# catid/siamese

Measured on AMD Instinct MI355X. Metric: device-resident GB/s encode+decode, 1400B pkts @20% loss; % HBM peak, higher is better.
Workload: dtype u8

## Files before the change

include/siamese_gpu.h:

```cpp
#ifndef SIAMESE_GPU_H
#define SIAMESE_GPU_H

#include "siamese.h"
#include <stddef.h>

#ifdef __cplusplus
extern "C" {
#endif

typedef struct SgpuEncoderImpl { int impl; }* SgpuEncoder;
typedef struct SgpuDecoderImpl { int impl; }* SgpuDecoder;

typedef struct SgpuRecoveryPacket
{
    const unsigned char* DeviceData;
    unsigned DataBytes;
    unsigned FooterBytes;
    unsigned char Footer[8];
    unsigned char Head[4];
    void* Producer;
} SgpuRecoveryPacket;

SIAMESE_EXPORT int sgpu_init(int device);

// ... 205 lines not shown
SIAMESE_EXPORT SiameseResult sgpu_decoders_ack_frames(const SgpuDecoder* decoders, unsigned count,
                                                      const unsigned* flows, unsigned byteLimit, void* deviceDst,
                                                      size_t stride, unsigned* deviceLens,
                                                      SiameseResult* results ,
                                                      unsigned* queuedOut);
SIAMESE_EXPORT SiameseResult sgpu_encoder_retransmit_frames(SgpuEncoder encoder, unsigned flow, unsigned maxPackets,
                                                            void* deviceDst, size_t stride, unsigned maxRows,
                                                            unsigned* deviceLens,
                                                            unsigned* packetNumsOut ,
                                                            unsigned* rowsOut, unsigned* framesOut);

#define SGPU_ROW_TRUNCATED       3
#define SGPU_PACKED_ACKS_DROPPED 0x20000000u

SIAMESE_EXPORT size_t sgpu_frames_duplex_bytes(unsigned count, unsigned maxFrames, unsigned ackSlots,
                                               unsigned ackBytes);
SIAMESE_EXPORT size_t sgpu_frames_duplex_slots(unsigned count, unsigned maxFrames);
SIAMESE_EXPORT long long sgpu_frames_scan_duplex(const void* deviceRows, size_t stride, const unsigned* deviceLens,
                                                 unsigned count, unsigned maxFrames, unsigned ackSlots,
                                                 unsigned ackBytes, void* pinnedOut);
SIAMESE_EXPORT SiameseResult sgpu_frames_recv_duplex(const SgpuDecoder* decoders, unsigned decoderCount,
                                                     const SgpuEncoder* encoders, unsigned encoderCount,
                                                     const void* heads, unsigned maxFrames, unsigned ackSlots,
                                                     unsigned ackBytes, const void* deviceRows, size_t stride,
                                                     unsigned count,
                                                     SiameseResult* results ,
                                                     unsigned* nextExpectedOut ,
                                                     unsigned* acceptedOut);

SIAMESE_EXPORT void sgpu_timing(int enable, int reset, double* execMs, double* totalMs);
SIAMESE_EXPORT void sgpu_timing_kernels(double* msOut, unsigned count);
SIAMESE_EXPORT void sgpu_engine_stats(uint64_t* out15);
SIAMESE_EXPORT void sgpu_engine_stats_ex(uint64_t* out, unsigned count);
SIAMESE_EXPORT void sgpu_measure_unique(int on);

SIAMESE_EXPORT uint64_t sgpu_arena_bytes(void);
SIAMESE_EXPORT int sgpu_arena_reserve(size_t bytes);

#ifdef __cplusplus
}
#endif

#endif
```

siamese_amd/csrc/backend.h:

```cpp
#pragma once

#include "ops.h"
#include <cstddef>
#include <cstdint>

namespace sgpu {

bool be_init(int device, const char** err);
const char* be_name();

void* be_dev_alloc(size_t bytes);
void be_dev_free(void* p);
void* be_host_alloc(size_t bytes);
void* be_host_alloc_mapped(size_t bytes);
void* be_host_device_ptr(void* host);
void be_host_free(void* p);

void be_h2d(void* dst, const void* src, size_t bytes);
void be_d2h(void* dst, const void* src, size_t bytes);
void be_memset(void* dst, int value, size_t bytes);
struct BeCopy
{
    uint64_t dst, src;
    uint64_t bytes;
// ... 5 lines not shown
struct BeIngest
{
    const IngestDesc* descs;
    uint32_t count;
    uint32_t maxBytes;
    const uint32_t* blocks = nullptr;
    uint32_t nblocks = 0;
};
void be_launch_ingest(const BeIngest& ingest);
void be_launch_exec(const void* stream, const ExecItem* items, uint32_t count, uint64_t* acct,
                    const uint32_t* results, uint32_t maxWindow);
uint32_t be_exec_stage_cap();
void be_launch_ldpc(const LdpcItem* items, uint32_t count, uint64_t* acct, const uint32_t* gates = nullptr,
                    const uint32_t* results = nullptr);
void be_launch_solve(const SolveDesc* solves, const SolveRow* rows, const uint8_t* coef, uint32_t* results,
                     const SolveItem* items, uint32_t count, uint32_t maxRows, uint64_t* acct,
                     uint32_t solveBegin, uint32_t solveCount);

struct BeGe
{
    const GeDesc* descs;
    const uint8_t* in;
    uint32_t count;
    uint32_t* results;
    const SolveRow* rowsIn;
    SolveRow* rows;
    uint8_t* coef;
    uint32_t maxRows, maxCols;
};
enum class GePlace
{
    kCodecStream,
    kSideStream,
};
void be_launch_ge(const BeGe& ge, GePlace place, const BeCopy& head = BeCopy{0, 0, 0});
void be_side_upload_ingest(const BeCopy& rest, const BeIngest& ingest);
void be_join_ge();

void be_launch_deliver(const DeliverItem* items, uint32_t count, uint32_t maxStride);
void be_launch_frame(const FrameItem* items, uint32_t count, uint32_t maxStride);
void be_launch_relay(const RelayItem* items, uint32_t count, uint32_t maxStride);
void be_launch_pack(const PackJob* jobs, uint32_t jobCount, const PackItem* items, uint32_t count, PlanRec* plan,
                    uint32_t maxStride);
void be_launch_concat(const ConcatJob* jobs, uint32_t jobCount, const ConcatItem* items, uint32_t count,
                      ConcatRec* recs, uint32_t maxBytes);

bool be_sync();

void* be_fence();
bool be_fence_wait(void* fence, unsigned spinUs, bool sleepPoll);

void* be_stage_h2d(void* dst, const void* src, size_t bytes);
void be_wait_mark(void* mark);
void be_mark_release(void* mark);
bool be_gather(const IngestDesc* descsHost, void* descsDev, uint32_t count, const void* devStage,
               void* hostOut, size_t bytes, void** packed, void** landed);
bool be_scan_rows(const void* rows, uint64_t stride, const uint32_t* lens, uint32_t count, void* devStage,
                  void* hostOut, void** packed, void** landed);
bool be_walk_rows(const void* rows, uint64_t stride, const uint32_t* lens, uint32_t count, uint32_t maxFrames,
                  void* devStage, void* hostOut, void** packed, void** landed);
bool be_ackwalk_rows(const void* rows, uint64_t stride, const uint32_t* lens, uint32_t count, uint32_t maxFrames,
                     uint32_t ackSlots, uint32_t ackBytes, void* devStage, void* hostOut, void** packed,
                     void** landed);
bool be_dense_rows(const void* rows, uint64_t stride, const uint32_t* lens, uint32_t count, uint32_t maxFrames,
                   uint32_t maxRecords, void* devStage, void* hostOut, void** packed, void** landed);
bool be_mark_sync(void* mark);
// ... 29 lines not shown
```

siamese_amd/csrc/backend_hip.hip:

```cpp
#include <hip/hip_runtime.h>

#include "backend.h"
#include "codedef.h"
#include "placement.h"
#include "pool.h"
#include "gf.h"

#include <algorithm>
#include <cctype>
#include <chrono>
#include <cstdlib>
#include <cstdio>
#include <string>
#include <type_traits>
#include <cstring>
#include <ctime>
#include <deque>
#include <mutex>
#include <vector>

namespace sgpu {


#define GMEM __attribute__((address_space(1)))
// ... 4112 lines not shown
                r0 = make_uint4((uint32_t)at, kRowOk | (type << 8) | ((h + inner) << 16) | (T << 24), flow, num);
                r1 = make_uint4(D, head, (uint32_t)tail, (uint32_t)(tail >> 32));
            }
        }
        if (!ok) {
            flags |= kPackedMalformed;
            break;
        }
        st16(rec + (uint64_t)n * 32, r0);
        st16(rec + (uint64_t)n * 32 + 16, r1);
        ++n;
        at += total;
    }
    for (uint32_t j = n; j < maxFrames; ++j) {
        st16(rec + (uint64_t)j * 32, make_uint4(0, 0, 0, 0));
        st16(rec + (uint64_t)j * 32 + 16, make_uint4(0, 0, 0, 0));
    }
    for (uint32_t a = acks; a < ackSlots; ++a)
        for (uint32_t o = 0; o < ackBytes; o += 16)
            st16(slot0 + (uint64_t)a * ackBytes + o, make_uint4(0, 0, 0, 0));
    *reinterpret_cast<GMEM uint32_t*>(out + (uint64_t)count * maxFrames * 32 + k * 4) = n | flags;
    if (k + 1 == count)
        for (uint64_t p = out + (uint64_t)count * maxFrames * 32 + (uint64_t)count * 4; p < slots; p += 4)
            *reinterpret_cast<GMEM uint32_t*>(p) = 0;
}


namespace {

hipStream_t g_stream = nullptr;
hipStream_t g_stageStream = nullptr;
hipStream_t g_gatherStream = nullptr;
hipStream_t g_geStream = nullptr;
hipEvent_t g_geFork = nullptr, g_geJoin = nullptr;
bool g_gePending = false;
bool g_ready = false;
int g_device = 0;

inline void bind_device()
{
    thread_local int bound = -1;
    if (bound != g_device) {
        (void)hipSetDevice(g_device);
        bound = g_device;
    }
}
bool g_timing = false;
uint32_t g_stageCap = 0;
double g_totalMs = 0;
double g_kernelMs[kBeKernelKinds] = {};

struct EvPair
{
    hipEvent_t a, b;
    BeKernel kind;
};
std::mutex g_evMu;
std::vector<EvPair> g_evFree;
std::deque<EvPair> g_evUsed;
std::vector<hipEvent_t> g_fenceFree;

EvPair take_events(BeKernel kind)
{
    EvPair e;
    {
        std::lock_guard<std::mutex> g(g_evMu);
        if (!g_evFree.empty()) {
// ... 90 lines not shown
        auto node_of = [](const char* b) {
            std::string s(b);
            for (char& c : s)
                c = (char)std::tolower((unsigned char)c);
            FILE* f = std::fopen(("/sys/bus/pci/devices/" + s + "/numa_node").c_str(), "r");
            int node = -1;
            if (f) {
                if (std::fscanf(f, "%d", &node) != 1)
                    node = -1;
                std::fclose(f);
            }
            return node;
        };
        if (hipDeviceGetPCIBusId(bus, sizeof(bus), cur) == hipSuccess) {
            const int myNode = node_of(bus);
            unsigned slice = 0;
            for (int d = 0; d < cur; ++d) {
                char other[64] = {0};
                if (hipDeviceGetPCIBusId(other, sizeof(other), d) == hipSuccess &&
                    node_of(other) == myNode)
                    ++slice;
            }
            place_near_device(bus, slice, WorkerPool::default_threads());
        }
    }
    if (hipStreamCreateWithFlags(&g_stream, hipStreamNonBlocking) != hipSuccess) {
        *err = "hipStreamCreate failed";
        return false;
    }
    if (hipStreamCreateWithFlags(&g_stageStream, hipStreamNonBlocking) != hipSuccess ||
        hipStreamCreateWithFlags(&g_gatherStream, hipStreamNonBlocking) != hipSuccess ||
        hipStreamCreateWithFlags(&g_geStream, hipStreamNonBlocking) != hipSuccess ||
        hipEventCreateWithFlags(&g_geFork, hipEventDisableTiming) != hipSuccess ||
        hipEventCreateWithFlags(&g_geJoin, hipEventDisableTiming) != hipSuccess) {
        *err = "hipStreamCreate (transfer streams) failed";
        return false;
    }
    if (!gf_init()) {
        *err = "GF(256) table self-check failed";
        return false;
    }
    static uint32_t perm[256][8];
    for (unsigned y = 0; y < 256; ++y) {
        uint8_t ta[8], tb[8], tc[4];
        for (unsigned k = 0; k < 8; ++k) {
            ta[k] = gf_mul((uint8_t)k, (uint8_t)y);
            tb[k] = gf_mul((uint8_t)(k << 3), (uint8_t)y);
        }
        for (unsigned k = 0; k < 4; ++k)
            tc[k] = gf_mul((uint8_t)(k << 6), (uint8_t)y);
        std::memset(perm[y], 0, sizeof(perm[y]));
        std::memcpy(&perm[y][0], ta, 8);
        std::memcpy(&perm[y][2], tb, 8);
        std::memcpy(&perm[y][4], tc, 4);
    }
    check(hipMemcpyToSymbol(HIP_SYMBOL(c_perm), perm, sizeof(perm)), "hipMemcpyToSymbol(perm)");
    check(hipMemcpyToSymbol(HIP_SYMBOL(c_inv), g_gf.inv, 256), "hipMemcpyToSymbol(inv)");
    check(hipMemcpyToSymbol(HIP_SYMBOL(c_sqr), g_gf.sqr, 256), "hipMemcpyToSymbol(sqr)");
    uint64_t pa[65], pg[65];
    pa[0] = 1;
    pg[0] = 0;
    for (unsigned j = 1; j <= 64; ++j) {
        pa[j] = pa[j - 1] * kPcgMul;
        pg[j] = pg[j - 1] * kPcgMul + 1;
    }
    check(hipMemcpyToSymbol(HIP_SYMBOL(c_pcgA), pa, sizeof(pa)), "hipMemcpyToSymbol(pcgA)");
    uint64_t ja[32], jg[32];
// ... 309 lines not shown
    hipLaunchKernelGGL(k_concat, dim3((count + kDeliverWaves - 1) / kDeliverWaves, chunks), dim3(64 * kDeliverWaves), 0,
                       g_stream, jobs, items, (const ConcatRec*)recs, count);
}

void be_launch_exec(const void* stream, const ExecItem* items, uint32_t count, uint64_t* acct,
                    const uint32_t* results, uint32_t maxWindow)
{
    if (count == 0)
        return;
    Timed t(kBeExec);
    uint32_t slots = 0;
    if (maxWindow != kNoRows)
        slots = kRowSums + (maxWindow < g_stageCap ? maxWindow : g_stageCap);
    hipLaunchKernelGGL(k_exec, dim3(count), dim3(kExecThreads), (size_t)(slots ? slots + 1 : 0) * kExecTileBytes,
                       g_stream, static_cast<const uint4*>(stream), items,
                       reinterpret_cast<unsigned long long*>(acct), results, slots);
}

void be_launch_ldpc(const LdpcItem* items, uint32_t count, uint64_t* acct, const uint32_t* gates,
                    const uint32_t* results)
{
    if (count == 0)
        return;
    Timed t(kBeLdpc);
    if (!gates)
        hipLaunchKernelGGL(k_ldpc<false>, dim3(count), dim3(64 * kLdpcWaves), 0, g_stream, items,
                           reinterpret_cast<unsigned long long*>(acct), (const uint32_t*)nullptr,
                           (const uint32_t*)nullptr);
    else
        hipLaunchKernelGGL(k_ldpc<true>, dim3(count), dim3(64 * kLdpcWaves), 0, g_stream, items,
                           reinterpret_cast<unsigned long long*>(acct), gates, results);
}

void be_launch_ge(const BeGe& ge, GePlace place, const BeCopy& head)
{
    if (ge.count == 0)
        return;
    check(hipEventRecord(g_geFork, g_stream), "hipEventRecord(ge fork)");
    check(hipStreamWaitEvent(g_geStream, g_geFork, 0), "hipStreamWaitEvent(ge fork)");
    const bool side = place == GePlace::kSideStream;
    hipStream_t stream = side ? g_geStream : g_stream;
    if (!side && head.bytes)
        check(hipMemcpyAsync((void*)(uintptr_t)head.dst, (const void*)(uintptr_t)head.src, head.bytes,
                             hipMemcpyHostToDevice, g_stream),
              "H2D (ge head)");
    {
        Timed t(kBeGe, stream);
        hipLaunchKernelGGL(k_ge, dim3(ge.count), dim3(kGeThreads), (size_t)ge_lds_bytes(ge.maxRows, ge.maxCols),
                           stream, ge.descs, ge.in, ge.results, ge.rows, ge.coef, ge.rowsIn);
    }
    if (side) {
        check(hipEventRecord(g_geJoin, g_geStream), "hipEventRecord(ge join)");
        g_gePending = true;
    }
}

void be_side_upload_ingest(const BeCopy& rest, const BeIngest& ingest)
{
    bind_device();
    if (rest.bytes)
        check(hipMemcpyAsync((void*)(uintptr_t)rest.dst, (const void*)(uintptr_t)rest.src, rest.bytes,
                             hipMemcpyHostToDevice, g_geStream),
              "H2D (upload rest)");
    launch_ingest(ingest, g_geStream);
    check(hipEventRecord(g_geJoin, g_geStream), "hipEventRecord(side join)");
    g_gePending = true;
}

void be_join_ge()
{
    if (!g_gePending)
        return;
    check(hipStreamWaitEvent(g_stream, g_geJoin, 0), "hipStreamWaitEvent(ge join)");
    g_gePending = false;
}

namespace {

enum SolvePath
{
    kPathSweeps = 0,
    kPathVector = 2,
};

void launch_solve(const SolveDesc* solves, const SolveRow* rows, const uint8_t* coef, uint32_t* results,
                  const SolveItem* items, uint32_t count, uint32_t maxRows, uint64_t* acct, uint32_t solveBegin,
                  uint32_t solveCount, SolvePath path)
{
    const uint32_t rowsCap = maxRows < kSolveLdsMaxRows ? maxRows : kSolveLdsMaxRows;
    const bool separate = solve_split(solveCount, maxRows);
    const bool tr = separate && path == kPathVector;
    unsigned long long* acctL = reinterpret_cast<unsigned long long*>(acct);
    const uint32_t prodCap = rowsCap < kProductMaxRows ? rowsCap : kProductMaxRows;
    if (tr) {
        hipLaunchKernelGGL(k_solve_pre, dim3(2 * solveCount), dim3(kPreThreads), (size_t)solve_pre_lds_bytes(rowsCap),
                           g_stream, solves + solveBegin, rows, coef, results, acctL, solveCount, 0u);
        hipLaunchKernelGGL(k_solve_tr, dim3(count * kTrSplit * kTrHalves), dim3(kTrThreads), (size_t)solve_tr_lds_bytes(prodCap),
                           g_stream, solves, rows, results, items);
    } else if (separate) {
        hipLaunchKernelGGL(k_solve_prefix, dim3(solveCount), dim3(64), (size_t)solve_prefix_lds_bytes(rowsCap),
                           g_stream, solves + solveBegin, rows, coef, results, acctL);
    }
    hipLaunchKernelGGL(k_solve_main, dim3(count), dim3(64 * kSolveWaves),
                       (size_t)solve_launch_lds_bytes(rowsCap, !separate), g_stream, solves, rows, coef, results,
                       items, acctL, (separate ? 1u : 0u) | (tr ? 4u : 0u));
}
// ... 531 lines not shown
```

siamese_amd/csrc/batch.cpp:

```cpp
#define SIAMESE_BUILDING
#include "../../include/siamese_gpu.h"

#include "backend.h"
#include "decoder.h"
#include "frames.h"
#include "encoder.h"
#include "engine.h"
#include "objpool.h"
#include "pool.h"

#include <algorithm>
#include <cstddef>
#include <cstdio>
#include <cstring>
#include <mutex>
#include <new>
#include <vector>

using namespace sgpu;

namespace {

bool g_batchReady = false;

// ... 1173 lines not shown
        *execMs = be_timing_kernel_ms(kBeExec);
    if (totalMs)
        *totalMs = be_timing_total_ms();
    if (reset)
        be_timing_reset();
}

SIAMESE_EXPORT void sgpu_timing_kernels(double* msOut, unsigned count)
{
    for (unsigned k = 0; k < count && k < kBeKernelKinds; ++k)
        msOut[k] = be_timing_kernel_ms((BeKernel)k);
}

SIAMESE_EXPORT void sgpu_engine_stats_ex(uint64_t* out, unsigned count)
{
    const EngineStats s = Engine::global()->stats();
    const Engine* e = Engine::global();
    const uint64_t v[37] = {s.flushes,    s.launches,    s.ops,        s.terms,    s.solves,
                            s.ingests,    s.uploadBytes, s.refOpBytes, s.outBytes, s.solveBytes,
                            s.assembleNs, s.waitNs,      s.completeNs, s.reclaimNs,
                            s.execLaunches, s.ldpcBytes, s.execUniqueBytes,
                            s.geJobs,     s.geChained,   s.geRetried,  s.geChainedWide,
                            s.delivers,   s.frames,      s.scans,      Engine::global()->walks(),
                            s.relays,     Engine::global()->packs(),
                            Engine::global()->duplexes(), Engine::global()->ack_frames(),
                            Engine::global()->concats(),
                            e->rows_shape(0), e->rows_shape(1), e->rows_shape(2), e->rows_shape(3),
                            e->rows_shape(4), be_exec_stage_cap(),
                            e->denses()};
    for (unsigned k = 0; k < count && k < 37; ++k)
        out[k] = v[k];
}

SIAMESE_EXPORT void sgpu_measure_unique(int on)
{
    Engine::set_measure_unique(on != 0);
}

SIAMESE_EXPORT void sgpu_engine_stats(uint64_t* out15)
{
    const EngineStats s = Engine::global()->stats();
    const uint64_t v[15] = {s.flushes,    s.launches,    s.ops,        s.terms,    s.solves,
                            s.ingests,    s.uploadBytes, s.refOpBytes, s.outBytes, s.solveBytes,
                            s.assembleNs, s.waitNs,      s.completeNs, s.reclaimNs,
                            s.execLaunches};
    std::memcpy(out15, v, sizeof(v));
}

SIAMESE_EXPORT uint64_t sgpu_arena_bytes(void)
{
    return Engine::global()->arena_bytes();
}

SIAMESE_EXPORT int sgpu_arena_reserve(size_t bytes)
{
    if (!g_batchReady)
        return -1;
    return Engine::global()->reserve(bytes) ? 0 : -1;
}

}
```

siamese_amd/csrc/engine.cpp:

```cpp
#include "engine.h"

#include <pthread.h>
#include "backend.h"
#include "codedef.h"
#include "pool.h"

#include <algorithm>
#include <chrono>
#include <cmath>
#include <cstdio>
#include <cstddef>
#include <cstdlib>
#include <cstring>

#ifndef SGPU_EXEC_LPT
#define SGPU_EXEC_LPT 1
#endif
#ifndef SGPU_EXEC_GROUPS
#define SGPU_EXEC_GROUPS 256
#endif

namespace sgpu {

void EngineStats::add(const EngineStats& o)
// ... 347 lines not shown
    op.n = R;
    op.valid = E;
    op.mix = U;
    op.termBegin = (uint32_t)(s.rowsData.size() / 16);
    op.termCount = words;
    s.ops.push_back(op);
    const size_t at = s.rowsData.size();
    s.rowsData.resize(at + (size_t)words * 16);
    uint8_t* w = s.rowsData.data() + at;
    std::memcpy(w, b.sums, sizeof(b.sums));
    w += sizeof(b.sums);
    std::memcpy(w, b.win.data(), (size_t)E * sizeof(WinEntry));
    w += (size_t)E * sizeof(WinEntry);
    std::memcpy(w, b.updates.data(), (size_t)U * sizeof(SumUpdate));
    w += (size_t)U * sizeof(SumUpdate);
    std::memcpy(w, b.rows.data(), (size_t)R * sizeof(RowItem));
    b.win.resize(winKept);
    s.rowsWords += words;
    if (b.maxExtent > s.maxExtent)
        s.maxExtent = b.maxExtent;
}


Program::~Program()
{
    if (!shard_) {
        if (b_)
            ProgramBody::put(b_);
        return;
    }
    Program* orphan = new Program(eng_, group_ | 2);
    orphan->shard_ = shard_;
    orphan->b_ = b_;
    b_ = nullptr;
    std::lock_guard<std::mutex> g(shard_->mu);
    auto it = std::find(shard_->dirty.begin(), shard_->dirty.end(), this);
    if (it != shard_->dirty.end())
        *it = orphan;
}

void Program::attach()
{
    if (!b_)
        b_ = ProgramBody::get();
    b_->group = group_ & 1;
    Shard& s = eng_->shard();
    shard_ = &s;
    std::lock_guard<std::mutex> g(s.mu);
    s.dirty.push_back(this);
}

void Program::lc_begin(uint64_t dst, uint32_t n, uint32_t valid, uint8_t mix)
{
    touch();
    if (b_->rb.open || !b_->copies.empty()) {
        b_->lc_seal();
        b_->rows_close();
    }
    if (b_->nsegs == 0)
        b_->new_segment();
    ProgramBody::Segment& s = b_->segs[b_->nsegs - 1];
    GfOp op;
    op.dst = dst;
    op.n = n;
    op.valid = valid < n ? valid : n;
    op.kind = OP_LINCOMB;
// ... 54 lines not shown
void Program::literal(uint64_t dst, uint32_t offset, const uint8_t* bytes, uint32_t len)
{
    if (len == 0)
        return;
    touch();
    if (!b_->lcb.items.empty()) {
        LcItem& it = b_->lcb.items.back();
        if (it.dst == dst && (it.mixLit >> 8) == 0 && len <= 8 && b_->lc_literal_fits(dst + offset, len)) {
            it.mixLit |= len << 8;
            it.litOffset = offset;
            std::memcpy(it.lit, bytes, len);
            ProgramBody::Segment& s = b_->segs[b_->nsegs - 1];
            if (offset + len > s.maxExtent)
                s.maxExtent = offset + len;
            return;
        }
    }
    b_->rows_close();
    if (b_->nsegs == 0)
        b_->new_segment();
    ProgramBody::Segment& s = b_->segs[b_->nsegs - 1];
    GfOp op;
    std::memset(&op, 0, sizeof(op));
    op.dst = dst;
    op.n = offset;
    op.valid = len;
    op.kind = OP_LITERAL;
    std::memcpy(op.lit, bytes, len);
    s.ops.push_back(op);
    if (offset + len > s.maxExtent)
        s.maxExtent = offset + len;
}

void Program::ingest_host(const DevBuf& dst, const void* data, uint32_t bytes, const uint8_t* hdr,
                          uint32_t hdrLen)
{
    eng_->stage_host_ingest(dst, data, bytes, hdr, hdrLen);
}

void Program::ingest_device(const DevBuf& dst, uint64_t src, uint32_t bytes, const uint8_t* hdr,
                            uint32_t hdrLen)
{
    ingest_run(dst.addr(), 0, src, 0, 1, bytes, hdr, hdrLen);
}

void Program::ingest_run(uint64_t dst, uint32_t dstStride, uint64_t src, uint32_t srcStride, uint32_t count,
                         uint32_t bytes, const uint8_t* hdr, uint32_t hdrLen)
{
    IngestDesc d;
    std::memset(&d, 0, sizeof(d));
    d.dst = dst;
    d.src = src;
    d.bytes = bytes;
    d.hdrLen = hdrLen;
    d.count = count;
    d.srcStride = count > 1 ? srcStride : 0;
    d.dstStride = count > 1 ? dstStride : 0;
    std::memcpy(d.hdr, hdr, hdrLen < 8 ? hdrLen : 8);
    eng_->add_ingest(d, -1);
}

uint32_t Program::solve(const std::vector<SolveRow>& rows, const uint8_t* coef, uint32_t maxBytes)
{
    SolveRow* r = nullptr;
    uint8_t* c = nullptr;
    solve_reserve((unsigned)rows.size(), &r, &c);
    std::memcpy(r, rows.data(), rows.size() * sizeof(SolveRow));
    std::memcpy(c, coef, rows.size() * rows.size());
    return solve_commit(maxBytes);
}

void Program::solve_reserve(unsigned m, SolveRow** rows, uint8_t** coef)
{
    touch();
    if (b_->nsegs == 0)
        b_->new_segment();
    if (b_->nsolves == b_->solves.size())
        b_->solves.emplace_back();
    ProgramBody::PendingSolve& ps = b_->solves[b_->nsolves];
    ps.rows.resize(m);
    ps.coef.resize((size_t)m * m);
    *rows = ps.rows.data();
    *coef = ps.coef.data();
}

uint32_t Program::solve_commit(uint32_t maxBytes, uint32_t gateWord)
{
    ProgramBody::PendingSolve& ps = b_->solves[b_->nsolves++];
    const size_t m = ps.rows.size();
    DevBuf head = eng_->alloc((uint32_t)m * 16u);
    if (head) {
// ... 328 lines not shown
    jb.count = count;
    jb.total = total;
    if (b_->concats.size() < (size_t)b_->nconcat + count)
        b_->concats.resize((size_t)b_->nconcat + count);
    for (uint32_t k = 0; k < count; ++k) {
        ConcatItem& it = b_->concats[b_->nconcat + k];
        it = items[k];
        it.job = b_->nconcatjob;
    }
    b_->nconcat += count;
    if (b_->nconcatjob == b_->concatJobs.size())
        b_->concatJobs.emplace_back();
    b_->concatJobs[b_->nconcatjob++] = jb;
}


bool Shard::Queues::empty() const
{
    if (!ingest.empty() || !downloads.empty())
        return false;
    for (const auto& r : released)
        if (!r.empty())
            return false;
    return true;
}

void Shard::Queues::clear()
{
    ingest.clear();
    hostStage.clear();
    downloads.clear();
    maxIngest = 0;
    pairCursor = 0;
    for (auto& r : released)
        r.clear();
}


Engine* Engine::global()
{
    static Engine e;
    return &e;
}

Engine::~Engine() { stop_threads(); }

bool Engine::init(int device, const char** err)
{
    if (ready_)
        return true;
    if (!be_init(device, err))
        return false;
    start_threads();
    ready_ = true;
    return true;
}

Shard& Engine::shard()
{
    thread_local Engine* owner = nullptr;
    thread_local Shard* mine = nullptr;
    if (owner != this) {
        std::lock_guard<std::mutex> g(shardsMu_);
        shards_.emplace_back(new Shard);
        mine = shards_.back().get();
        owner = this;
// ... 46 lines not shown
    if (bytes < 64)
        return 64;
    if (bytes <= 4096)
        return (bytes + 63) & ~63u;
    if (bytes <= 131072)
        return (bytes + 1023) & ~1023u;
    return (bytes + 65535) & ~65535u;
}

namespace {

size_t cap_class(uint32_t cap)
{
    if (cap <= 4096)
        return cap / 64 - 1;
    if (cap <= 131072)
        return 64 + cap / 1024 - 5;
    return 188 + cap / 65536 - 3;
}

constexpr size_t kChunkBytes = 64u << 20;
constexpr size_t kRegionBytes = 4u << 20;
constexpr size_t kMagazine = 512;
constexpr size_t kMaxMagazine = 512;
constexpr size_t kRefillBytes = 1u << 20;

}

uint8_t* Engine::carve_region(size_t bytes)
{
    std::lock_guard<std::mutex> g(arenaMu_);
    if (bytes > kChunkBytes / 4) {
        arenaBytes_ += bytes;
        return (uint8_t*)be_dev_alloc(bytes);
    }
    if (chunks_.empty() || chunks_.back().used + bytes > chunks_.back().size) {
        if (!spare_.empty()) {
            chunks_.push_back(spare_.back());
            spare_.pop_back();
        } else {
            uint8_t* base = (uint8_t*)be_dev_alloc(kChunkBytes);
            if (!base)
                return nullptr;
            arenaBytes_ += kChunkBytes;
            chunks_.push_back(Chunk{base, kChunkBytes, 0});
        }
    }
    Chunk& c = chunks_.back();
    uint8_t* p = c.base + c.used;
    c.used += bytes;
    return p;
}

bool Engine::reserve(size_t bytes)
{
    std::lock_guard<std::mutex> g(arenaMu_);
    size_t have = 0;
    for (const Chunk& c : spare_)
        have += c.size;
    while (have < bytes) {
        uint8_t* base = (uint8_t*)be_dev_alloc(kChunkBytes);
        if (!base)
            return false;
        arenaBytes_ += kChunkBytes;
        spare_.push_back(Chunk{base, kChunkBytes, 0});
        have += kChunkBytes;
    }
// ... 343 lines not shown
    size_t oFrame = 0, nFrame = 0;
    uint32_t maxFrameStride = 0;
    size_t oRelay = 0, nRelay = 0;
    uint32_t maxRelayStride = 0;
    size_t oPackJob = 0, nPackJob = 0;
    size_t oPack = 0, nPack = 0;
    size_t oPlan = 0;
    uint32_t maxPackStride = 0;
    size_t oConcatJob = 0, nConcatJob = 0;
    size_t oConcat = 0, nConcat = 0;
    size_t oConcatRec = 0;
    uint32_t maxConcatBytes = 0;
    size_t oCopy = 0;
    uint64_t wideBase = 0;
    bool wideGated = false;
    size_t oWideGate = 0;
    bool wideZero = false;
    uint32_t resultWords = 0;
    std::vector<const Shard::Download*> dls;
    std::vector<BeCopy> copies;
    uint8_t* upBase = nullptr;
    EngineStats st;
    void* fence = nullptr;
    bool launched = false;
    std::vector<uint32_t> resultBase[2];
    struct Download
    {
        void* host;
        size_t off;
        uint32_t bytes;
    };
    std::vector<Download> downloads;
    std::vector<void*> marks;
    bool assembled = false;
};

namespace {

const bool g_timeline = std::getenv("SGPU_TIMELINE") != nullptr;
void tl(const char* what, uint64_t ticket)
{
    if (g_timeline)
        std::fprintf(stderr, "eng %10.3f ms  %s t%llu\n", (double)now_ns() / 1e6, what,
                     (unsigned long long)ticket);
}

constexpr size_t kAcctBytes = 32;

constexpr size_t kParallelWords = 1u << 16;
#ifndef SGPU_SEAL_CHUNK
#define SGPU_SEAL_CHUNK 32
#endif
#ifndef SGPU_SEG_CHUNK
#define SGPU_SEG_CHUNK 16
#endif
#ifndef SGPU_INGEST_CHUNK
#define SGPU_INGEST_CHUNK 8192
#endif
#ifndef SGPU_SOLVE_CHUNK
#define SGPU_SOLVE_CHUNK 64
#endif

std::atomic<bool> g_measureUnique{false};

struct Range
{
// ... 95 lines not shown
        launcher_loop();
    });
    completer_ = std::thread([this] {
        pthread_setname_np(pthread_self(), "sgpu-complete");
        completer_loop();
    });
}

void Engine::stop_threads()
{
    {
        std::lock_guard<std::mutex> g(qMu_);
        stop_ = true;
    }
    launchCv_.notify_all();
    completeCv_.notify_all();
    setCv_.notify_all();
    doneCv_.notify_all();
    if (launcher_.joinable())
        launcher_.join();
    if (completer_.joinable())
        completer_.join();
}

Batch* Engine::take_batch()
{
    std::vector<Shard*> shards;
    {
        std::lock_guard<std::mutex> g(shardsMu_);
        for (auto& s : shards_)
            shards.push_back(s.get());
    }
    Batch* b = nullptr;
    for (Shard* s : shards) {
        if (s->dirty.empty() && s->q.empty())
            continue;
        if (!b)
            b = new Batch;
        for (Program* p : s->dirty) {
            ProgramBody* body = p->b_;
            p->b_ = nullptr;
            p->shard_ = nullptr;
            if (body) {
                if (body->empty() && body->callbacks.empty())
                    ProgramBody::put(body);
                else
                    b->bodies[body->group].push_back(body);
            }
            if (p->group_ & 2)
                delete p;
        }
        s->dirty.clear();
        if (!s->q.empty()) {
            Shard::Queues next;
            {
                std::lock_guard<std::mutex> g(s->mu);
                if (!s->spare.empty()) {
                    next = std::move(s->spare.back());
                    s->spare.pop_back();
                }
            }
            b->queues.push_back(std::move(s->q));
            b->queueOwner.push_back(s);
            s->q = std::move(next);
        }
    }
    if (!b)
        return nullptr;
    const uint64_t ticket = ++nextTicket_;
    tl("enqueue", ticket);
    b->ticket = ticket;
    b->set = (unsigned)(ticket % kSets);
    {
        std::lock_guard<std::mutex> g(qMu_);
        b->marks.swap(pendingMarks_);
    }
    return b;
}


uint64_t Engine::enqueue()
{
    if (failed())
        return 0;
    std::lock_guard<std::mutex> sub(submitMu_);
    Batch* b = take_batch();
    if (!b)
        return nextTicket_;
    const uint64_t ticket = b->ticket;
    {
        std::lock_guard<std::mutex> g(qMu_);
        toLaunch_.push_back(b);
        queuedSeen_.fetch_add(1, std::memory_order_release);
    }
// ... 569 lines not shown
        xs.wideUsed += need;
    }
    if (tBytes) {
        ensure_solve(xs, tBytes);
        const uint64_t tBase = (uint64_t)(uintptr_t)xs.solveDev;
        for (SolveDesc& d : sdescs)
            if (d.tinv) {
                d.tinv = tBase + (d.tinv - 1);
                d.xout = tBase + (d.xout - 1);
            }
    }

    uint8_t* up = xs.upHost;
    const uint64_t stageDev = (uint64_t)(uintptr_t)(bt.upBase + oStage);
    constexpr size_t kSegChunk = SGPU_SEG_CHUNK;
    constexpr size_t kSolveChunk = SGPU_SOLVE_CHUNK;
    struct Task
    {
        int kind;
        size_t a, b;
    };
    std::vector<Task> tasks;
    for (size_t i = 0; i < segs.size(); i += kSegChunk)
        tasks.push_back(Task{0, i, std::min(segs.size(), i + kSegChunk)});
    for (size_t i = 0; i < grefs.size(); i += kSolveChunk)
        tasks.push_back(Task{3, i, std::min(grefs.size(), i + kSolveChunk)});
    for (size_t i = 0; i < srefs.size(); i += kSolveChunk)
        tasks.push_back(Task{2, i, std::min(srefs.size(), i + kSolveChunk)});
    for (size_t qi = 0; qi < bt.queues.size(); ++qi)
        for (size_t c = 0; c < std::max<size_t>(1, bt.queues[qi].ingest.size()); c += kIngestChunk)
            tasks.push_back(Task{1, qi, c});
    const bool measureUnique = measure_unique();
    std::atomic<uint64_t> uniqueBytes{0};
    run(tasks.size(), [&](size_t ti) {
        const Task& t = tasks[ti];
        if (t.kind == 0) {
            if (measureUnique) {
                std::vector<Range> rd, wr;
                uint64_t u = 0;
                for (size_t si = t.a; si < t.b; ++si)
                    u += segment_unique_bytes(*segs[si].seg, rd, wr);
                uniqueBytes.fetch_add(u, std::memory_order_relaxed);
            }
            for (size_t si = t.a; si < t.b; ++si) {
                const SegRef& r = segs[si];
                const ProgramBody::Segment& s = *r.seg;
                uint8_t* w = up + bt.oStream + (size_t)r.wordBase * 16;
                size_t wi = 0;
                LdpcItem* wItem = (LdpcItem*)(up + bt.oWide) + r.wideBase;
                uint32_t* wGate = bt.wideGated ? (uint32_t*)(up + bt.oWideGate) + r.wideBase : nullptr;
                uint64_t wOff = bt.wideBase + r.wideOff;
                size_t gi = 0;
                for (uint32_t oi = 0; oi < (uint32_t)s.ops.size(); ++oi) {
                    const GfOp& op = s.ops[oi];
                    std::memcpy(w, &op, sizeof(GfOp));
                    uint32_t opGate = 0;
                    if (op.kind != OP_LITERAL) {
                        while (gi < s.gates.size() && s.gates[gi].opEnd <= oi)
                            ++gi;
                        const bool gated = gi < s.gates.size() && s.gates[gi].opBegin <= oi;
                        opGate = gated ? 1u + s.gates[gi].word + r.resultBase : 0u;
                        reinterpret_cast<GfOp*>(w)->termBegin = opGate;
                    }
                    w += sizeof(GfOp);
                    if (op.kind == OP_ROWS || op.kind == OP_COPIES || op.kind == OP_LINCOMBS) {
                        const size_t bytes = (size_t)op.termCount * 16;
// ... 42 lines not shown
                for (uint32_t t = 0; t < tiles; t += r.tilesPerItem)
                    items[n++] = ExecItem{r.wordBase, r.words, nOpsSeg,
                                          exec_tiles(t, std::min(r.tilesPerItem, tiles - t))};
            }
        } else if (t.kind == 3) {
            for (size_t i = t.a; i < t.b; ++i) {
                uint8_t* in = up + bt.oGeIn + grefs[i].inOff;
                if (grefs[i].cancelled) {
                    std::memset(in, 0, ge_input_bytes(1, 1, 0));
                    GeRow* r = reinterpret_cast<GeRow*>(in);
                    r->kind = GE_PARITY;
                    r->colCount = 1;
                    continue;
                }
                std::memcpy(in, grefs[i].g->in.data(), grefs[i].g->in.size());
            }
        } else if (t.kind == 2) {
            for (size_t i = t.a; i < t.b; ++i) {
                const SolveRef& r = srefs[i];
                std::memcpy(up + bt.oSR + r.rowBase * sizeof(SolveRow), r.ps->rows.data(),
                            r.ps->rows.size() * sizeof(SolveRow));
                std::memcpy(up + bt.oCoef + r.coefBase, r.ps->coef.data(), r.ps->coef.size());
            }
        } else {
            const Shard::Queues& q = bt.queues[t.a];
            IngestDesc* descs = (IngestDesc*)(up + bt.oIngD) + descBase[t.a];
            const size_t end = std::min(q.ingest.size(), t.b + kIngestChunk);
            uint32_t* blk = t.b < q.ingest.size() ? (uint32_t*)(up + bt.oIngB) + blockBase[t.a][t.b / kIngestChunk]
                                                  : nullptr;
            for (size_t i = t.b; i < end; ++i) {
                IngestDesc d = q.ingest[i].d;
                if (q.ingest[i].hostOffset >= 0)
                    d.src = stageDev + stageBase[t.a] + (uint64_t)q.ingest[i].hostOffset;
                descs[i] = d;
                const uint32_t di = (uint32_t)(descBase[t.a] + i);
                const uint32_t n = d.count ? d.count : 1u;
                for (uint32_t g = 0; g * kIngestWaves < n; ++g)
                    *blk++ = di << 4 | g;
            }
            if (t.b == 0 && !q.hostStage.empty())
                std::memcpy(up + oStage + stageBase[t.a], q.hostStage.data(), q.hostStage.size());
        }
    });
    if (!sdescs.empty()) {
        std::memcpy(up + bt.oSD, sdescs.data(), sdescs.size() * sizeof(SolveDesc));
        std::memcpy(up + bt.oSI, sitems.data(), sitems.size() * sizeof(SolveItem));
    }
    if (!gdescs.empty())
        std::memcpy(up + bt.oGeD, gdescs.data(), gdescs.size() * sizeof(GeDesc));
    if (nDeliver) {
        DeliverItem* di = (DeliverItem*)(up + bt.oDeliver);
        uint32_t max16 = 0;
        for (int g = 0; g < 2; ++g)
            for (const ProgramBody* p : bt.bodies[g]) {
                if (p->ndeliver == 0)
                    continue;
                std::memcpy(di, p->delivers.data(), p->ndeliver * sizeof(DeliverItem));
                for (uint32_t k = 0; k < p->ndeliver; ++k)
                    max16 = std::max(max16, di[k].stride16);
                di += p->ndeliver;
            }
        bt.maxDeliverStride = (uint32_t)std::min<uint64_t>((uint64_t)max16 << 4, 0xffffffffu);
    }
    if (nFrame) {
        FrameItem* fi = (FrameItem*)(up + bt.oFrame);
        uint32_t max16 = 0;
        size_t litBase = 0;
        for (int g = 0; g < 2; ++g)
            for (const ProgramBody* p : bt.bodies[g]) {
                if (p->nframe == 0)
                    continue;
                std::memcpy(fi, p->frames.data(), p->nframe * sizeof(FrameItem));
                for (uint32_t k = 0; k < p->nframe; ++k)
                    max16 = std::max(max16, fi[k].stride16);
                if (!p->frameLit.empty()) {
                    std::memcpy(up + oFrameLit + litBase, p->frameLit.data(), p->frameLit.size());
// ... 82 lines not shown
                                bt.dls[i]->bytes});
        if (xs.downHostDev) {
            BeCopy* dl = (BeCopy*)(up + bt.oCopy);
            const uint64_t shift = (uint64_t)(uintptr_t)xs.downHostDev - (uint64_t)(uintptr_t)xs.downHost;
            for (size_t i = 0; i < cp.size(); ++i)
                dl[i] = BeCopy{cp[i].dst + shift, cp[i].src, cp[i].bytes};
        }
    }

    st.flushes = 1;
    st.launches = phases.size() + (nIngest ? 1 : 0) + (gdescs.empty() ? 0 : 1) + (nDeliver ? 1 : 0) +
                  (nFrame ? 1 : 0) + (nRelay ? 1 : 0) + (nPackJob ? 1 : 0) + (nPack ? 1 : 0) +
                  (nConcatJob ? 1 : 0) + (nConcat ? 1 : 0);
    for (unsigned k = 0; k < kRowsShapeStats; ++k)
        if (rowsShape[k])
            rowsShape_[k].fetch_add(rowsShape[k], std::memory_order_relaxed);
    st.delivers = nDeliver;
    st.frames = nFrame;
    st.relays = nRelay;
    st.ops = nOps;
    st.terms = nTerms;
    st.solves = sdescs.size();
    st.ingests = nIngest;
    st.uploadBytes = bt.upBytes;
    st.execUniqueBytes = uniqueBytes.load(std::memory_order_relaxed);
    st.assembleNs = now_ns() - t0;
}

void Engine::launch_batch(Batch& bt)
{
    XferSet& xs = sets_[bt.set];
    EngineStats& st = bt.st;

    for (void* m : bt.marks) {
        be_wait_mark(m);
        be_mark_release(m);
    }
    bt.marks.clear();
    const bool copyUp = bt.upBytes && bt.upBase == xs.upDev;
    const size_t head = (copyUp && bt.nGe) ? bt.geHead : 0;
    uint64_t* acctDev = (uint64_t*)xs.downDev;
    uint32_t* resultsDev = (uint32_t*)(xs.downDev + kAcctBytes);
    const BeCopy rest{(uint64_t)(uintptr_t)xs.upDev + head, (uint64_t)(uintptr_t)xs.upHost + head,
                      bt.upBytes - head};
    const BeIngest ingest{(const IngestDesc*)(bt.upBase + bt.oIngD), (uint32_t)bt.nIngest, bt.maxIngest,
                          (const uint32_t*)(bt.upBase + bt.oIngB), (uint32_t)bt.nIngBlocks};
    auto ge_at = [&](const uint8_t* up) {
        return BeGe{(const GeDesc*)(up + bt.oGeD), up + bt.oGeIn, (uint32_t)bt.nGe, resultsDev,
                    (const SolveRow*)(up + bt.oSR), (SolveRow*)(bt.upBase + bt.oSR), bt.upBase + bt.oCoef,
                    bt.geMaxRows, bt.geMaxCols};
    };
    if (head && bt.allGated && xs.upHostDev) {
        be_launch_ge(ge_at(xs.upHostDev), GePlace::kCodecStream);
        be_side_upload_ingest(rest, ingest);
    } else if (head) {
        be_launch_ge(ge_at(bt.upBase), GePlace::kCodecStream,
                     BeCopy{(uint64_t)(uintptr_t)xs.upDev, (uint64_t)(uintptr_t)xs.upHost, head});
        be_side_upload_ingest(rest, ingest);
    } else {
        if (bt.nGe)
            be_launch_ge(ge_at(bt.upBase), GePlace::kSideStream);
        if (copyUp)
            be_copy_pinned(&rest, 1, true);
        be_launch_ingest(ingest);
    }
    const bool ingested = head != 0;
    if (xs.acctZero) {
        be_memset(acctDev, 0, 4 * sizeof(uint64_t));
        xs.acctZero = false;
    }
    if (bt.wideZero)
        be_memset(xs.wideDev, 0, xs.wideCap);
    size_t wideDone = 0;
    for (size_t k = 0; k < bt.phases.size() && bt.phases[k].kind == Phase::EXEC; ++k)
        wideDone = bt.phases[k].wideBegin + bt.phases[k].wideCount;
    const uint32_t* wideGates = bt.wideGated ? (const uint32_t*)(bt.upBase + bt.oWideGate) : nullptr;
    if (wideDone) {
        if (ingested || wideGates)
            be_join_ge();
        be_launch_ldpc((const LdpcItem*)(bt.upBase + bt.oWide), (uint32_t)wideDone, acctDev + 3, wideGates,
                       resultsDev);
    }
    for (const Phase& ph : bt.phases) {
        be_join_ge();
        if (ph.kind == Phase::EXEC) {
            if (ph.wideCount && ph.wideBegin >= wideDone)
                be_launch_ldpc((const LdpcItem*)(bt.upBase + bt.oWide) + ph.wideBegin, (uint32_t)ph.wideCount,
                               acctDev + 3, wideGates ? wideGates + ph.wideBegin : nullptr, resultsDev);
            be_launch_exec(bt.upBase + bt.oStream, (const ExecItem*)(bt.upBase + bt.oItems) + ph.itemBegin,
// ... 392 lines not shown
```

siamese_amd/csrc/engine.h:

```cpp
#pragma once

#include "ops.h"

#include <atomic>
#include <condition_variable>
#include <cstdint>
#include <cstdio>
#include <cstdlib>
#include <deque>
#include <functional>
#include <memory>
#include <mutex>
#include <pthread.h>
#include <shared_mutex>
#include <thread>
#include <vector>

namespace sgpu {

class InstanceLock
{
public:
    InstanceLock() = default;
    InstanceLock(const InstanceLock&) = delete;
// ... 361 lines not shown
    {
        if (b_)
            b_->rows_close();
    }

    void copy(uint64_t dst, uint64_t src, uint32_t len);

    void deliver(uint64_t src, uint32_t cap, uint64_t dst, uint64_t lenOut, uint64_t stride);

    void frame(uint64_t src, uint32_t bytes, const uint8_t* hdr, uint32_t hdrLen, uint64_t dst, uint64_t lenOut,
               uint64_t stride, uint32_t lenBase = 0);
    void frame_literal(const uint8_t* data, uint32_t bytes, const uint8_t* hdr, uint32_t hdrLen, uint64_t dst,
                       uint64_t lenOut, uint64_t stride);

    void relay(uint64_t src, uint32_t cap, uint32_t flow, uint32_t packetNum, uint64_t dst, uint64_t lenOut,
               uint64_t stride);

    void pack(const PackItem* items, uint32_t count, uint64_t rows, uint64_t stride, uint32_t maxRows, uint64_t lens,
              uint64_t info);

    void concat(const ConcatItem* items, uint32_t count, uint32_t total, uint64_t dst, uint32_t capacity,
                uint64_t offsets, uint64_t info);

    bool empty() const { return !b_ || b_->empty(); }

private:
    friend class Engine;
    void touch()
    {
        if (!shard_)
            attach();
    }
    void attach();
    void rows_open(uint32_t base, bool keepWindow) { b_->rows_open(base, keepWindow); }

    Engine* eng_;
    int group_;
    Shard* shard_ = nullptr;
    ProgramBody* b_ = nullptr;
};

struct EngineStats
{
    uint64_t flushes = 0, launches = 0, ops = 0, terms = 0, solves = 0, ingests = 0;
    uint64_t uploadBytes = 0;
    uint64_t refOpBytes = 0, outBytes = 0;
    uint64_t solveBytes = 0;
    uint64_t ldpcBytes = 0;
    uint64_t assembleNs = 0, waitNs = 0, completeNs = 0, reclaimNs = 0;
    uint64_t execLaunches = 0;
    uint64_t execUniqueBytes = 0;
    uint64_t geJobs = 0, geChained = 0, geRetried = 0;
    uint64_t geChainedWide = 0;
    uint64_t delivers = 0;
    uint64_t frames = 0;
    uint64_t scans = 0;
    uint64_t relays = 0;

    void add(const EngineStats& o);
};

class Engine
{
public:
    static Engine* global();
    ~Engine();

    bool init(int device, const char** err);
    bool ready() const { return ready_; }

// ... 162 lines not shown
    void ensure_wide(XferSet& x, size_t bytes);
    void ensure_solve(XferSet& x, size_t bytes);
    void ensure_down(XferSet& x, size_t bytes);

    uint8_t* gUpHost_ = nullptr;
    uint8_t* gUpDev_ = nullptr;
    size_t gUpCap_ = 0;
    uint8_t* gHost_ = nullptr;
    uint8_t* gDev_ = nullptr;
    size_t gCap_ = 0;
    static constexpr unsigned kGatherSlots = 4;
    struct GatherSlot
    {
        uint8_t* upHost = nullptr;
        uint8_t* upDev = nullptr;
        size_t upCap = 0;
        uint8_t* stage = nullptr;
        size_t stageCap = 0;
        void* landed = nullptr;
        int64_t ticket = 0;
    } gslots_[kGatherSlots];
    int64_t gNext_ = 0;
    bool gather_land(GatherSlot& g);
    int64_t rows_async(const void* rows, uint64_t stride, const uint32_t* lens, unsigned count, unsigned maxFrames,
                       void* pinnedOut, unsigned ackSlots = 0, unsigned ackBytes = 0, unsigned maxRecords = 0);
    std::atomic<uint64_t> walks_{0};
    std::atomic<uint64_t> packs_{0};
    std::atomic<uint64_t> duplexes_{0};
    std::atomic<uint64_t> ackFrames_{0};
    std::atomic<uint64_t> concats_{0};
    std::atomic<uint64_t> denses_{0};
    static constexpr unsigned kRowsShapeStats = 5;
    std::atomic<uint64_t> rowsShape_[kRowsShapeStats] = {};

public:
    uint64_t rows_shape(unsigned k) const { return rowsShape_[k].load(std::memory_order_relaxed); }
    uint64_t walks() const { return walks_.load(std::memory_order_relaxed); }
    uint64_t packs() const { return packs_.load(std::memory_order_relaxed); }
    uint64_t concats() const { return concats_.load(std::memory_order_relaxed); }
    uint64_t denses() const { return denses_.load(std::memory_order_relaxed); }
    uint64_t duplexes() const { return duplexes_.load(std::memory_order_relaxed); }
    uint64_t ack_frames() const { return ackFrames_.load(std::memory_order_relaxed); }
    void count_ack_frames(uint64_t n) { ackFrames_.fetch_add(n, std::memory_order_relaxed); }
};

struct Shard
{
    struct IngestRec
    {
        IngestDesc d;
        int64_t hostOffset;
    };
    struct Download
    {
        void* host;
        uint64_t dev;
        uint32_t bytes;
    };
    struct Queues
    {
        std::vector<IngestRec> ingest;
        std::vector<uint8_t> hostStage;
        std::vector<Download> downloads;
        std::vector<std::vector<uint8_t*>> released;
        uint32_t maxIngest = 0;
        size_t pairCursor = 0;
        bool empty() const;
        void clear();
    };

    std::mutex mu;
    std::vector<Program*> dirty;
    Queues q;
    std::vector<Queues> spare;
    std::vector<std::vector<uint8_t*>> freeLists;
    uint8_t* bump = nullptr;
    size_t bumpLeft = 0;
    int64_t inUse = 0;
    EngineStats stats;
};

}
```

Baseline: 4212.

## Launch GE prologue early on side stream when prior batches' dependencies are done

Adds a kSideEarly placement that launches the GE kernel and its head H2D on the side stream without forking from the codec stream. It applies when per-program ticket tracking shows the batch's inputs do not depend on in-flight work, no arena-sourced ingest or caller writes are pending, and no marks exist. The goal is to overlap the Gaussian-elimination prologue with earlier batches still on the codec stream. The price is extra host bookkeeping (ticket stamps, an arena range scan) and ordering risk if the dependency tracking misses a hazard; the join event is double-buffered so the waits stay correct.

```diff
diff --git a/include/siamese_gpu.h b/include/siamese_gpu.h
--- a/include/siamese_gpu.h
+++ b/include/siamese_gpu.h
@@ -261,6 +261,7 @@
 SIAMESE_EXPORT void sgpu_timing_kernels(double* msOut, unsigned count);
 SIAMESE_EXPORT void sgpu_engine_stats(uint64_t* out15);
 SIAMESE_EXPORT void sgpu_engine_stats_ex(uint64_t* out, unsigned count);
+SIAMESE_EXPORT uint64_t sgpu_engine_early_prologues(void);
 SIAMESE_EXPORT void sgpu_measure_unique(int on);
 
 SIAMESE_EXPORT uint64_t sgpu_arena_bytes(void);
diff --git a/siamese_amd/csrc/backend.h b/siamese_amd/csrc/backend.h
--- a/siamese_amd/csrc/backend.h
+++ b/siamese_amd/csrc/backend.h
@@ -61,6 +61,7 @@
 {
     kCodecStream,
     kSideStream,
+    kSideEarly,
 };
 void be_launch_ge(const BeGe& ge, GePlace place, const BeCopy& head = BeCopy{0, 0, 0});
 void be_side_upload_ingest(const BeCopy& rest, const BeIngest& ingest);
diff --git a/siamese_amd/csrc/backend_hip.hip b/siamese_amd/csrc/backend_hip.hip
--- a/siamese_amd/csrc/backend_hip.hip
+++ b/siamese_amd/csrc/backend_hip.hip
@@ -4168,7 +4168,8 @@
 hipStream_t g_stageStream = nullptr;
 hipStream_t g_gatherStream = nullptr;
 hipStream_t g_geStream = nullptr;
-hipEvent_t g_geFork = nullptr, g_geJoin = nullptr;
+hipEvent_t g_geFork = nullptr, g_geJoin[2] = {nullptr, nullptr};
+unsigned g_geJoinAt = 0;
 bool g_gePending = false;
 bool g_ready = false;
 int g_device = 0;
@@ -4325,7 +4326,8 @@
         hipStreamCreateWithFlags(&g_gatherStream, hipStreamNonBlocking) != hipSuccess ||
         hipStreamCreateWithFlags(&g_geStream, hipStreamNonBlocking) != hipSuccess ||
         hipEventCreateWithFlags(&g_geFork, hipEventDisableTiming) != hipSuccess ||
-        hipEventCreateWithFlags(&g_geJoin, hipEventDisableTiming) != hipSuccess) {
+        hipEventCreateWithFlags(&g_geJoin[0], hipEventDisableTiming) != hipSuccess ||
+        hipEventCreateWithFlags(&g_geJoin[1], hipEventDisableTiming) != hipSuccess) {
         *err = "hipStreamCreate (transfer streams) failed";
         return false;
     }
@@ -4701,27 +4703,39 @@
                            reinterpret_cast<unsigned long long*>(acct), gates, results);
 }
 
+namespace {
+
+void record_ge_join(const char* what)
+{
+    g_geJoinAt ^= 1u;
+    check(hipEventRecord(g_geJoin[g_geJoinAt], g_geStream), what);
+    g_gePending = true;
+}
+
+}
+
 void be_launch_ge(const BeGe& ge, GePlace place, const BeCopy& head)
 {
     if (ge.count == 0)
         return;
-    check(hipEventRecord(g_geFork, g_stream), "hipEventRecord(ge fork)");
-    check(hipStreamWaitEvent(g_geStream, g_geFork, 0), "hipStreamWaitEvent(ge fork)");
-    const bool side = place == GePlace::kSideStream;
+    const bool early = place == GePlace::kSideEarly;
+    if (!early) {
+        check(hipEventRecord(g_geFork, g_stream), "hipEventRecord(ge fork)");
+        check(hipStreamWaitEvent(g_geStream, g_geFork, 0), "hipStreamWaitEvent(ge fork)");
+    }
+    const bool side = place != GePlace::kCodecStream;
     hipStream_t stream = side ? g_geStream : g_stream;
-    if (!side && head.bytes)
+    if (place != GePlace::kSideStream && head.bytes)
         check(hipMemcpyAsync((void*)(uintptr_t)head.dst, (const void*)(uintptr_t)head.src, head.bytes,
-                             hipMemcpyHostToDevice, g_stream),
+                             hipMemcpyHostToDevice, stream),
               "H2D (ge head)");
     {
         Timed t(kBeGe, stream);
         hipLaunchKernelGGL(k_ge, dim3(ge.count), dim3(kGeThreads), (size_t)ge_lds_bytes(ge.maxRows, ge.maxCols),
                            stream, ge.descs, ge.in, ge.results, ge.rows, ge.coef, ge.rowsIn);
     }
-    if (side) {
-        check(hipEventRecord(g_geJoin, g_geStream), "hipEventRecord(ge join)");
-        g_gePending = true;
-    }
+    if (side)
+        record_ge_join("hipEventRecord(ge join)");
 }
 
 void be_side_upload_ingest(const BeCopy& rest, const BeIngest& ingest)
@@ -4732,15 +4746,14 @@
                              hipMemcpyHostToDevice, g_geStream),
               "H2D (upload rest)");
     launch_ingest(ingest, g_geStream);
-    check(hipEventRecord(g_geJoin, g_geStream), "hipEventRecord(side join)");
-    g_gePending = true;
+    record_ge_join("hipEventRecord(side join)");
 }
 
 void be_join_ge()
 {
     if (!g_gePending)
         return;
-    check(hipStreamWaitEvent(g_stream, g_geJoin, 0), "hipStreamWaitEvent(ge join)");
+    check(hipStreamWaitEvent(g_stream, g_geJoin[g_geJoinAt], 0), "hipStreamWaitEvent(ge join)");
     g_gePending = false;
 }
 
diff --git a/siamese_amd/csrc/batch.cpp b/siamese_amd/csrc/batch.cpp
--- a/siamese_amd/csrc/batch.cpp
+++ b/siamese_amd/csrc/batch.cpp
@@ -1229,6 +1229,11 @@
         out[k] = v[k];
 }
 
+SIAMESE_EXPORT uint64_t sgpu_engine_early_prologues(void)
+{
+    return Engine::global()->early_prologues();
+}
+
 SIAMESE_EXPORT void sgpu_measure_unique(int on)
 {
     Engine::set_measure_unique(on != 0);
diff --git a/siamese_amd/csrc/engine.cpp b/siamese_amd/csrc/engine.cpp
--- a/siamese_amd/csrc/engine.cpp
+++ b/siamese_amd/csrc/engine.cpp
@@ -403,6 +403,7 @@
     Program* orphan = new Program(eng_, group_ | 2);
     orphan->shard_ = shard_;
     orphan->b_ = b_;
+    orphan->lastTicket_ = lastTicket_;
     b_ = nullptr;
     std::lock_guard<std::mutex> g(shard_->mu);
     auto it = std::find(shard_->dirty.begin(), shard_->dirty.end(), this);
@@ -523,9 +524,39 @@
         s.maxExtent = offset + len;
 }
 
+namespace {
+
+inline uint64_t ticket_before(uint64_t next, uint32_t low)
+{
+    if (low == 0)
+        return 0;
+    const uint64_t back = (uint32_t)((uint32_t)next - low);
+    return back < next ? next - back : 0;
+}
+
+inline uint32_t stamp_of(uint64_t ticket)
+{
+    return (uint32_t)ticket ? (uint32_t)ticket : 1u;
+}
+
+}
+
+void Program::note_ingest()
+{
+    if (shard_)
+        return;
+    const uint64_t next = eng_->nextTicket_.load(std::memory_order_relaxed) + 1;
+    if (lastTicket_ == stamp_of(next))
+        return;
+    Shard::Queues& q = eng_->shard().q;
+    q.prevTicket = std::max(q.prevTicket, ticket_before(next, lastTicket_));
+    lastTicket_ = stamp_of(next);
+}
+
 void Program::ingest_host(const DevBuf& dst, const void* data, uint32_t bytes, const uint8_t* hdr,
                           uint32_t hdrLen)
 {
+    note_ingest();
     eng_->stage_host_ingest(dst, data, bytes, hdr, hdrLen);
 }
 
@@ -548,6 +579,7 @@
     d.srcStride = count > 1 ? srcStride : 0;
     d.dstStride = count > 1 ? dstStride : 0;
     std::memcpy(d.hdr, hdr, hdrLen < 8 ? hdrLen : 8);
+    note_ingest();
     eng_->add_ingest(d, -1);
 }
 
@@ -942,6 +974,7 @@
     downloads.clear();
     maxIngest = 0;
     pairCursor = 0;
+    prevTicket = 0;
     for (auto& r : released)
         r.clear();
 }
@@ -1054,7 +1087,10 @@
     std::lock_guard<std::mutex> g(arenaMu_);
     if (bytes > kChunkBytes / 4) {
         arenaBytes_ += bytes;
-        return (uint8_t*)be_dev_alloc(bytes);
+        uint8_t* base = (uint8_t*)be_dev_alloc(bytes);
+        if (base)
+            large_.push_back(Chunk{base, bytes, bytes});
+        return base;
     }
     if (chunks_.empty() || chunks_.back().used + bytes > chunks_.back().size) {
         if (!spare_.empty()) {
@@ -1464,6 +1500,8 @@
     };
     std::vector<Download> downloads;
     std::vector<void*> marks;
+    uint64_t prevTicket = 0;
+    bool ingestFromArena = false;
     bool assembled = false;
 };
 
@@ -1625,12 +1663,16 @@
             shards.push_back(s.get());
     }
     Batch* b = nullptr;
+    const uint64_t mine = nextTicket_.load(std::memory_order_relaxed) + 1;
     for (Shard* s : shards) {
         if (s->dirty.empty() && s->q.empty())
             continue;
         if (!b)
             b = new Batch;
         for (Program* p : s->dirty) {
+            if (p->lastTicket_ != stamp_of(mine))
+                b->prevTicket = std::max(b->prevTicket, ticket_before(mine, p->lastTicket_));
+            p->lastTicket_ = stamp_of(mine);
             ProgramBody* body = p->b_;
             p->b_ = nullptr;
             p->shard_ = nullptr;
@@ -1653,6 +1695,7 @@
                     s->spare.pop_back();
                 }
             }
+            b->prevTicket = std::max(b->prevTicket, s->q.prevTicket);
             b->queues.push_back(std::move(s->q));
             b->queueOwner.push_back(s);
             s->q = std::move(next);
@@ -2288,6 +2331,19 @@
             tasks.push_back(Task{1, qi, c});
     const bool measureUnique = measure_unique();
     std::atomic<uint64_t> uniqueBytes{0};
+    std::vector<std::pair<uint64_t, uint64_t>> arena;
+    uint64_t arenaLo = ~0ull, arenaHi = 0;
+    if (nIngest && !gdescs.empty() && bt.marks.empty()) {
+        std::lock_guard<std::mutex> g(arenaMu_);
+        for (const std::vector<Chunk>* v : {&chunks_, &spare_, &large_})
+            for (const Chunk& c : *v) {
+                const uint64_t lo = (uint64_t)(uintptr_t)c.base;
+                arena.emplace_back(lo, lo + c.size);
+                arenaLo = std::min(arenaLo, lo);
+                arenaHi = std::max(arenaHi, lo + c.size);
+            }
+    }
+    std::atomic<bool> fromArena{false};
     run(tasks.size(), [&](size_t ti) {
         const Task& t = tasks[ti];
         if (t.kind == 0) {
@@ -2396,6 +2452,14 @@
                 IngestDesc d = q.ingest[i].d;
                 if (q.ingest[i].hostOffset >= 0)
                     d.src = stageDev + stageBase[t.a] + (uint64_t)q.ingest[i].hostOffset;
+                else {
+                    const uint64_t lo = d.src;
+                    const uint64_t hi = lo + (uint64_t)((d.count ? d.count : 1u) - 1) * d.srcStride + d.bytes;
+                    if (lo < arenaHi && hi > arenaLo)
+                        for (const auto& r : arena)
+                            if (lo < r.second && hi > r.first)
+                                fromArena.store(true, std::memory_order_relaxed);
+                }
                 descs[i] = d;
                 const uint32_t di = (uint32_t)(descBase[t.a] + i);
                 const uint32_t n = d.count ? d.count : 1u;
@@ -2406,6 +2470,7 @@
                 std::memcpy(up + oStage + stageBase[t.a], q.hostStage.data(), q.hostStage.size());
         }
     });
+    bt.ingestFromArena = fromArena.load(std::memory_order_relaxed);
     if (!sdescs.empty()) {
         std::memcpy(up + bt.oSD, sdescs.data(), sdescs.size() * sizeof(SolveDesc));
         std::memcpy(up + bt.oSI, sitems.data(), sitems.size() * sizeof(SolveItem));
@@ -2554,6 +2619,7 @@
     XferSet& xs = sets_[bt.set];
     EngineStats& st = bt.st;
 
+    const bool marked = !bt.marks.empty();
     for (void* m : bt.marks) {
         be_wait_mark(m);
         be_mark_release(m);
@@ -2572,11 +2638,19 @@
                     (const SolveRow*)(up + bt.oSR), (SolveRow*)(bt.upBase + bt.oSR), bt.upBase + bt.oCoef,
                     bt.geMaxRows, bt.geMaxCols};
     };
+    const uint64_t done = doneSeen_.load(std::memory_order_acquire);
+    const bool early = head && !marked && !bt.ingestFromArena && done + 1 < bt.ticket && bt.prevTicket <= done &&
+                       callerWriteTicket_.load(std::memory_order_relaxed) <= done;
+    const GePlace place = early ? GePlace::kSideEarly : GePlace::kCodecStream;
+    if (early)
+        earlyPrologues_.fetch_add(1, std::memory_order_relaxed);
+    if (bt.nDeliver || bt.nFrame || bt.nRelay || bt.nPackJob || bt.nConcatJob)
+        callerWriteTicket_.store(bt.ticket, std::memory_order_relaxed);
     if (head && bt.allGated && xs.upHostDev) {
-        be_launch_ge(ge_at(xs.upHostDev), GePlace::kCodecStream);
+        be_launch_ge(ge_at(xs.upHostDev), place);
         be_side_upload_ingest(rest, ingest);
     } else if (head) {
-        be_launch_ge(ge_at(bt.upBase), GePlace::kCodecStream,
+        be_launch_ge(ge_at(bt.upBase), place,
                      BeCopy{(uint64_t)(uintptr_t)xs.upDev, (uint64_t)(uintptr_t)xs.upHost, head});
         be_side_upload_ingest(rest, ingest);
     } else {
diff --git a/siamese_amd/csrc/engine.h b/siamese_amd/csrc/engine.h
--- a/siamese_amd/csrc/engine.h
+++ b/siamese_amd/csrc/engine.h
@@ -417,10 +417,12 @@
             attach();
     }
     void attach();
+    void note_ingest();
     void rows_open(uint32_t base, bool keepWindow) { b_->rows_open(base, keepWindow); }
 
     Engine* eng_;
     int group_;
+    uint32_t lastTicket_ = 0;
     Shard* shard_ = nullptr;
     ProgramBody* b_ = nullptr;
 };
@@ -649,8 +651,12 @@
     std::atomic<uint64_t> denses_{0};
     static constexpr unsigned kRowsShapeStats = 5;
     std::atomic<uint64_t> rowsShape_[kRowsShapeStats] = {};
+    std::atomic<uint64_t> earlyPrologues_{0};
+    std::atomic<uint64_t> callerWriteTicket_{0};
+    std::vector<Chunk> large_;
 
 public:
+    uint64_t early_prologues() const { return earlyPrologues_.load(std::memory_order_relaxed); }
     uint64_t rows_shape(unsigned k) const { return rowsShape_[k].load(std::memory_order_relaxed); }
     uint64_t walks() const { return walks_.load(std::memory_order_relaxed); }
     uint64_t packs() const { return packs_.load(std::memory_order_relaxed); }
@@ -682,6 +688,7 @@
         std::vector<std::vector<uint8_t*>> released;
         uint32_t maxIngest = 0;
         size_t pairCursor = 0;
+        uint64_t prevTicket = 0;
         bool empty() const;
         void clear();
     };
```

Result: slower. 4064 (-3.5%).
